# karapostK/hassaku

Measured on AMD Instinct MI355X. Metric: BPR triplets/sec, higher is better.
Workload: dtype f32

## Files before the change

hassaku_amd/csrc/hsk_fwd_part.h:

```cpp
#pragma once
#include "hsk_sampler.h"
#include "hsk_sort.h"
#include "hsk_step_kernels.h"

struct hsk_ride_fwd {
  int n_total;
  hsk_ride_sort Bk;
  hsk_ride_sample S;
  hsk_ride_sort R;
};
struct hsk_ride_item {
  int n_total;
  hsk_ride_sort C;
  hsk_ride_sort H;
};

struct hsk_part_args {
  int n_part;
  int n_items;
  int n_ahead_blocks;
  int ahead_stride;
};
#define HSK_PART_LIST_MAX 256

__device__ __forceinline__ void hsk_ride_fwd_roles(const hsk_ride_fwd& rf, int bid) {
  if (bid < rf.Bk.n_blocks) {
    __shared__ int bucket_lds[5 * HSK_PIPE_MAX_IPB + 2];
    hsk_sort_bucket_body(rf.Bk.perm1, rf.Bk.n_entries, rf.Bk.n_items, rf.Bk.plan, rf.Bk.bstart, rf.Bk.perm, rf.Bk.offsets,
                         nullptr, nullptr, bid, bucket_lds);
    return;
  }
  bid -= rf.Bk.n_blocks;
  if (bid < rf.S.n_blocks) {
    hsk_ride_sample_body(rf.S, bid);
    return;
  }
  bid -= rf.S.n_blocks;
  if (bid < rf.R.n_blocks) hsk_sort_rowscan_body(rf.R.hist, rf.R.plan, rf.R.btot, bid);
}

template <int V, int NCH, bool FULL, int R, int LOSS, bool GEN>
__global__ __launch_bounds__(256) void k_fwd_part(const float* __restrict__ Uw, const float* __restrict__ Iw,
                                                  const float* __restrict__ Ib, const int* __restrict__ u32,
                                                  const int* __restrict__ it32, int B, int K , int D, float inv_norm,
                                                  float* __restrict__ g_s, float* __restrict__ dUp,
                                                  double* __restrict__ loss_p, hsk_lazy_user_args lz, hsk_part_args pa,
                                                  hsk_ahead_args aa, hsk_ride_fwd rf) {
  static_assert(LOSS == HSK_LOSS_BPR || LOSS == HSK_LOSS_BCE, "the sampled softmax needs all negatives in one wave");
  int bid = (int)blockIdx.x;
  if (bid < rf.n_total) {
    hsk_ride_fwd_roles(rf, bid);
    return;
  }
  bid -= rf.n_total;
  if (pa.ahead_stride > 0) {
    const int o = bid >> 3, r = bid & 7, n_ao = pa.n_ahead_blocks >> 3;
    const int period = pa.ahead_stride + 1, full = n_ao * period;
    if (o < full) {
      const int k = o / period, j = o - k * period;
      if (j == pa.ahead_stride) {
        hsk_user_ahead_body<V, NCH, FULL, GEN>(aa, k * 8 + r);
        return;
      }
      bid = (k * pa.ahead_stride + j) * 8 + r;
    } else {
      bid = (n_ao * pa.ahead_stride + (o - full)) * 8 + r;
    }
  } else {
    if (bid < pa.n_ahead_blocks) {
      hsk_user_ahead_body<V, NCH, FULL, GEN>(aa, bid);
      return;
    }
    bid -= pa.n_ahead_blocks;
  }
  const int lane = hsk_lane();
  const int wave = hsk_uniform_i(threadIdx.x >> 6);
  const int P = pa.n_part, M = 8 / P;
  const int xcd = bid & 7, q = xcd / M, sx = xcd - q * M, t = bid >> 3;
  const int b = (t * M + sx) * 4 + wave;
  if (b >= B) return;

  using Row = hsk_row<V, NCH>;
  const int* __restrict__ irow = it32 + (long long)b * K;
  const int u_v = u32[b];
  const int i0_v = irow[0];
  int idv[HSK_PART_LIST_MAX / 64];
#pragma unroll
  for (int r = 0; r < HSK_PART_LIST_MAX / 64; ++r) {
    const int c = P + r * 64 + lane;
    idv[r] = (c < K) ? irow[c] : -1;
  }
  const int u = hsk_uniform_i(u_v);
  const int i0 = hsk_uniform_i(i0_v);
  Row ur, r0, acc;
  hsk_row_load<V, NCH, FULL>(ur, Uw + (long long)u * D, lane, D);
  hsk_row_load<V, NCH, FULL>(r0, Iw + (long long)i0 * D, lane, D);
  int done_v = 0, own_v = 0;
  if (lz.mU) {
    done_v = lz.last_step[u];
    own_v = lz.owner[u];
  }
  const float bias0 = Ib ? Ib[i0] : 0.f;
  __shared__ int lst_id[4][HSK_PART_LIST_MAX], lst_col[4][HSK_PART_LIST_MAX];
  const int lo = (int)(((long long)q * pa.n_items + P - 1) / P), hi = (int)(((long long)(q + 1) * pa.n_items + P - 1) / P);
  int n_mine = 0;
#pragma unroll
  for (int r = 0; r < HSK_PART_LIST_MAX / 64; ++r) {
    const bool mine = idv[r] >= lo && idv[r] < hi;
    const unsigned long long m = __ballot(mine);
    if (mine) {
      const int pos = n_mine + __popcll(m & ((1ull << lane) - 1ull));
      lst_id[wave][pos] = idv[r];
      lst_col[wave][pos] = P + r * 64 + lane;
    }
    n_mine += __popcll(m);
  }
  __builtin_amdgcn_wave_barrier();

  int kc = 0;
  int nr = min(64, n_mine);
  int myidx = (lane < nr) ? lst_id[wave][lane] : i0;
  int mycol = (lane < nr) ? lst_col[wave][lane] : 0;
  Row bufA[R], bufB[R];
  auto prefetch = [&](Row(&buf)[R], int j) {
#pragma unroll
    for (int r = 0; r < R; ++r)
      if (j + r < nr)
        hsk_row_load<V, NCH, FULL>(buf[r], Iw + (long long)hsk_readlane_i(myidx, j + r) * D, lane, D);
  };
  prefetch(bufA, 0);
  float mybias = Ib ? Ib[myidx] : 0.f;

  if (lz.mU)
    hsk_user_row_current<V, NCH, FULL>(ur, u, b, B, D, lane, lz, q == 0, hsk_uniform_i(done_v), hsk_uniform_i(own_v));
  else if (lz.ucur && q == 0)
    hsk_row_store<V, NCH, FULL>(ur, lz.ucur + (long long)b * D, lane, D);
  hsk_row_zero(acc);
  const float s0 = hsk_wave_sum(hsk_row_dot_partial(ur, r0)) + bias0;

  float gsum = 0.f;
  double lsum = 0.0;
  while (true) {
    float gv = 0.f, xv = 0.f;
    auto process = [&](Row(&buf)[R], int j) {
      hsk_weigh_rows<LOSS>(ur, buf, j, nr, lane, mybias, s0, inv_norm, acc, gsum, gv, xv);
    };
    for (int j = 0; j < nr; j += 2 * R) {
      prefetch(bufB, j + R);
      process(bufA, j);
      prefetch(bufA, j + 2 * R);
      process(bufB, j + R);
    }
    if (lane < nr) {
      g_s[(long long)b * K + mycol] = gv;
      lsum += (double)hsk_softplus(LOSS == HSK_LOSS_BPR ? -xv : xv);
    }
    kc += 64;
    if (kc >= n_mine) break;
    nr = min(64, n_mine - kc);
    myidx = (lane < nr) ? lst_id[wave][kc + lane] : i0;
    mycol = (lane < nr) ? lst_col[wave][kc + lane] : 0;
    prefetch(bufA, 0);
    mybias = Ib ? Ib[myidx] : 0.f;
  }
  float gp;
  if (LOSS == HSK_LOSS_BPR) {
    gp = gsum;
  } else {
    gp = (q == 0) ? inv_norm / (1.f + expf(s0)) : 0.f;
    if (q == 0 && lane == 0) lsum += (double)hsk_softplus(-s0);
  }
  hsk_row_axpy(acc, -gp, r0);
  hsk_row_store<V, NCH, FULL>(acc, dUp + ((long long)b * P + q) * D, lane, D);
  const double l = hsk_wave_sum_f64(lsum);
  if (lane == 0) {
    g_s[(long long)b * K + q] = -gp;
    loss_p[(long long)q * B + b] = l;
  }
}
```

hassaku_amd/csrc/hsk_item_sliced.h:

```cpp
#pragma once
#include "hsk_rows.h"
#include "hsk_step_kernels.h"
#include "hsk_fwd_part.h"

#ifndef HSK_ITEM_MLP
#define HSK_ITEM_MLP 4
#endif
#ifndef HSK_ITEM_NT
#define HSK_ITEM_NT 0
#endif
template <int VS>
__device__ __forceinline__ hsk_vec<VS> hsk_ldg_stream(const float* p) {
#if HSK_ITEM_NT
  hsk_vec<VS> r;
#pragma unroll
  for (int i = 0; i < VS; ++i) r.v[i] = __builtin_nontemporal_load(p + i);
  return r;
#else
  return hsk_ldg<VS>(p);
#endif
}
template <int VS>
__device__ __forceinline__ void hsk_stg_stream(float* p, const hsk_vec<VS>& x) {
#if HSK_ITEM_NT
#pragma unroll
  for (int i = 0; i < VS; ++i) __builtin_nontemporal_store(x.v[i], p + i);
#else
  hsk_stg<VS>(p, x);
#endif
}

#ifdef HSK_DEBUG_XCC
__device__ unsigned hsk_dbg_xcc[64];
#endif
struct hsk_item_args {
  const float* Uw;
  float* Iw; float* Ib; float* mI; float* vI; float* mIb; float* vIb;
  const int* u32;
  const float* g_s; const int* perm; const int* offsets;
  int n_items, K, D, n_slices_pad, items_per_wave;
  hsk_adamw_consts c;
  float* gI_out; float* gIb_out;
  const int* touched; const int* n_touched; int* last_step_i; int step;
  const int* pend;
  const hsk_step_desc* desc; int rel;
  const float2* ctab; int ctab_len;
  int n_part;
};

template <bool PART>
__device__ __forceinline__ float hsk_entry_weight(const hsk_item_args& a, int e, int bpos) {
  float g = a.g_s[e];
  if (PART && e == bpos * a.K)
    for (int q = 1; q < a.n_part; ++q) g += a.g_s[e + q];
  return g;
}

template <bool APPLY, int VS, bool GEN, bool LAZY, bool PART = false>
__device__ __forceinline__ void hsk_item_sliced_body(const hsk_item_args& a, int bid) {
  const float* __restrict__ Uw = a.Uw;
  float* __restrict__ Iw = a.Iw;
  float* __restrict__ Ib = a.Ib;
  float* __restrict__ mI = a.mI;
  float* __restrict__ vI = a.vI;
  float* __restrict__ mIb = a.mIb;
  float* __restrict__ vIb = a.vIb;
  const int* __restrict__ u32 = a.u32;
  const float* __restrict__ g_s = a.g_s;
  const int* __restrict__ perm = a.perm;
  const int* __restrict__ offsets = a.offsets;
  const int n_items = a.n_items, K = a.K, D = a.D, n_slices_pad = a.n_slices_pad, items_per_wave = a.items_per_wave;
  hsk_adamw_consts c = a.c;
  int step = a.step;
  hsk_resolve_step(a.desc, a.rel, a.ctab, a.ctab_len, step, c);
  float* __restrict__ gI_out = a.gI_out;
  float* __restrict__ gIb_out = a.gIb_out;
  const int* __restrict__ touched = a.touched;
  const int* __restrict__ n_touched = a.n_touched;
  int* __restrict__ last_step_i = a.last_step_i;
  const int lane = hsk_lane();
  const int wave = hsk_uniform_i(threadIdx.x >> 6);
  int slice, group;
  if (n_slices_pad < 8) {
    const int xcd = bid & 7, r = bid >> 3;
    slice = xcd % n_slices_pad;
    group = r * (8 / n_slices_pad) + xcd / n_slices_pad;
  } else {
    slice = bid % n_slices_pad;
    group = bid / n_slices_pad;
  }
  constexpr int SW = 64 * VS;
  const int d = slice * SW + lane * VS;
  const bool live = d < D;
  if (slice * SW >= D) return;
  const int first = (group * 4 + wave) * items_per_wave;
  const int n_list = LAZY ? hsk_uniform_i(*n_touched) : n_items;
  for (int t = 0; t < items_per_wave; ++t) {
    const int idx = first + t;
    if (idx >= n_list) return;
    const int i = LAZY ? hsk_uniform_i(touched[idx]) : idx;
    const int beg = hsk_uniform_i(offsets[i]);
    const int end = hsk_uniform_i(offsets[i + 1]);
    hsk_vec<VS> p = hsk_zero<VS>(), m = hsk_zero<VS>(), v = hsk_zero<VS>();
    if (APPLY && live) {
      p = hsk_ldg_stream<VS>(Iw + (long long)i * D + d);
      m = hsk_ldg_stream<VS>(mI + (long long)i * D + d);
      v = hsk_ldg_stream<VS>(vI + (long long)i * D + d);
    }
    hsk_vec<VS> acc = hsk_zero<VS>();
    float gb_lane = 0.f;
    for (int c0 = beg; c0 < end; c0 += 64) {
      const int nr = min(64, end - c0);
      int myu = 0;
      float myg = 0.f;
      if (lane < nr) {
        const int e = perm[c0 + lane];
        const int bpos = e / K;
        myg = PART ? hsk_entry_weight<true>(a, e, bpos) : g_s[e];
        myu = u32 ? u32[bpos] : bpos;
      }
      gb_lane += myg;
      for (int j = 0; j < nr; j += HSK_ITEM_MLP) {
        hsk_vec<VS> val[HSK_ITEM_MLP];
#pragma unroll
        for (int r = 0; r < HSK_ITEM_MLP; ++r)
          val[r] = (j + r < nr && live) ? hsk_ldg<VS>(Uw + (long long)hsk_readlane_i(myu, min(j + r, 63)) * D + d)
                                        : hsk_zero<VS>();
#pragma unroll
        for (int r = 0; r < HSK_ITEM_MLP; ++r)
          if (j + r < nr) {
            const float g = hsk_readlane_f(myg, j + r);
#pragma unroll
            for (int q = 0; q < VS; ++q) acc.v[q] = fmaf(g, val[r].v[q], acc.v[q]);
          }
      }
    }
    if (APPLY) {
      const int behind = (LAZY && !GEN && a.pend) ? (step - 1) - hsk_uniform_i(a.pend[idx]) : 0;
      for (int r = 0; r < behind; ++r) {
#pragma unroll
        for (int q = 0; q < VS; ++q) {
          m.v[q] = fmaf(c.w1, -m.v[q], m.v[q]);
          v.v[q] = v.v[q] * c.beta2;
        }
      }
      if (live) {
#pragma unroll
        for (int q = 0; q < VS; ++q) hsk_adamw_update<GEN>(p.v[q], m.v[q], v.v[q], acc.v[q], c);
        hsk_stg_stream<VS>(Iw + (long long)i * D + d, p);
        hsk_stg_stream<VS>(mI + (long long)i * D + d, m);
        hsk_stg_stream<VS>(vI + (long long)i * D + d, v);
      }
      if (slice == 0 && Ib) {
        const float gbias = hsk_wave_sum(gb_lane);
        if (lane == 0) {
          float pb = Ib[i], mb = mIb[i], vb = vIb[i];
          for (int r = 0; r < behind; ++r) {
            mb = fmaf(c.w1, -mb, mb);
            vb = vb * c.beta2;
          }
          hsk_adamw_update<GEN>(pb, mb, vb, gbias, c);
          Ib[i] = pb;
          mIb[i] = mb;
          vIb[i] = vb;
        }
      }
      if (LAZY && slice == 0 && lane == 0) last_step_i[i] = step;
    } else {
      if (live) hsk_stg<VS>(gI_out + (long long)i * D + d, acc);
      if (slice == 0 && gIb_out) {
        const float gbias = hsk_wave_sum(gb_lane);
        if (lane == 0) gIb_out[i] = gbias;
      }
    }
  }
}

template <int V, int NCH, bool FULL, bool GEN, bool LAZY>
__device__ __forceinline__ void hsk_item_row_body(const hsk_item_args& a, int bid) {
  const int lane = hsk_lane();
  const int idx = bid * 4 + hsk_uniform_i(threadIdx.x >> 6);
  const int n_list = LAZY ? hsk_uniform_i(*a.n_touched) : a.n_items;
  if (idx >= n_list) return;
  hsk_adamw_consts c = a.c;
  int step = a.step;
  hsk_resolve_step(a.desc, a.rel, a.ctab, a.ctab_len, step, c);
  const int i = LAZY ? hsk_uniform_i(a.touched[idx]) : idx;
  const int D = a.D, K = a.K;
  using Row = hsk_row<V, NCH>;
  const int beg = hsk_uniform_i(a.offsets[i]);
  const int end = hsk_uniform_i(a.offsets[i + 1]);
  float* prow = a.Iw + (long long)i * D;
  float* mrow = a.mI + (long long)i * D;
  float* vrow = a.vI + (long long)i * D;
  Row p, m, v, acc;
  hsk_row_load<V, NCH, FULL>(p, prow, lane, D);
  hsk_row_load<V, NCH, FULL>(m, mrow, lane, D);
  hsk_row_load<V, NCH, FULL>(v, vrow, lane, D);
  float pb = 0.f, mb = 0.f, vb = 0.f;
  if (a.Ib && lane == 0) {
    pb = a.Ib[i];
    mb = a.mIb[i];
    vb = a.vIb[i];
  }
  hsk_row_zero(acc);
  float gb_lane = 0.f;
  for (int c0 = beg; c0 < end; c0 += 64) {
    const int nr = min(64, end - c0);
    int myu = 0;
    float myg = 0.f;
    if (lane < nr) {
      const int e = a.perm[c0 + lane];
      myg = a.g_s[e];
      myu = a.u32 ? a.u32[e / K] : e / K;
    }
    gb_lane += myg;
    for (int j = 0; j < nr; j += 4) {
      Row buf[4];
#pragma unroll
      for (int r = 0; r < 4; ++r)
        if (j + r < nr) hsk_row_load<V, NCH, FULL>(buf[r], a.Uw + (long long)hsk_readlane_i(myu, min(j + r, 63)) * D, lane, D);
#pragma unroll
      for (int r = 0; r < 4; ++r)
        if (j + r < nr) hsk_row_axpy(acc, hsk_readlane_f(myg, j + r), buf[r]);
    }
  }
  const int behind = (LAZY && !GEN && a.pend) ? (step - 1) - hsk_uniform_i(a.pend[idx]) : 0;
  for (int r = 0; r < behind; ++r) {
#pragma unroll
    for (int cc = 0; cc < NCH; ++cc)
#pragma unroll
      for (int q = 0; q < V; ++q) {
        m.c[cc].v[q] = fmaf(c.w1, -m.c[cc].v[q], m.c[cc].v[q]);
        v.c[cc].v[q] = v.c[cc].v[q] * c.beta2;
      }
    mb = fmaf(c.w1, -mb, mb);
    vb = vb * c.beta2;
  }
#pragma unroll
  for (int cc = 0; cc < NCH; ++cc)
#pragma unroll
    for (int q = 0; q < V; ++q) hsk_adamw_update<GEN>(p.c[cc].v[q], m.c[cc].v[q], v.c[cc].v[q], acc.c[cc].v[q], c);
  hsk_row_store<V, NCH, FULL>(p, prow, lane, D);
  hsk_row_store<V, NCH, FULL>(m, mrow, lane, D);
  hsk_row_store<V, NCH, FULL>(v, vrow, lane, D);
  if (a.Ib) {
    const float gbias = hsk_wave_sum(gb_lane);
    if (lane == 0) {
      hsk_adamw_update<GEN>(pb, mb, vb, gbias, c);
      a.Ib[i] = pb;
      a.mIb[i] = mb;
      a.vIb[i] = vb;
    }
  }
  if (LAZY && lane == 0) a.last_step_i[i] = step;
}

template <bool APPLY, int VS, bool GEN, bool LAZY = false, bool PART = false>
__global__ __launch_bounds__(256) void k_item_update_sliced(hsk_item_args a, const int* __restrict__ g_ovf = nullptr,
                                                            const int* __restrict__ g_poison = nullptr) {
  if (APPLY && hsk_guard_skip(g_ovf, g_poison)) return;
  hsk_item_sliced_body<APPLY, VS, GEN, LAZY, PART>(a, (int)blockIdx.x);
}

template <int V, int NCH, bool FULL, bool GEN, bool LAZY>
__global__ __launch_bounds__(256) void k_item_update_rows(hsk_item_args a, const int* __restrict__ g_ovf = nullptr,
                                                          const int* __restrict__ g_poison = nullptr) {
  if (hsk_guard_skip(g_ovf, g_poison)) return;
  hsk_item_row_body<V, NCH, FULL, GEN, LAZY>(a, (int)blockIdx.x);
}

template <int V, int NCH, bool FULL, int VS, bool GEN, bool LAZYI, bool PART = false>
__global__ __launch_bounds__(256) __attribute__((amdgpu_waves_per_eu(8, 8)))
void k_item_user(hsk_item_args ia, hsk_user_lazy_args ua, int n_user_blocks, int dense_users, hsk_ahead_args aa,
                 int n_ahead_blocks, hsk_ride_item ri = hsk_ride_item{}) {
  int bid = (int)blockIdx.x;
  if (PART) {
    if (bid < ri.n_total) {
      __shared__ int ride_lds[HSK_SORT_SCATTER_LDS];
      if (bid < ri.C.n_blocks) {
        hsk_sort_scatter_body(ri.C.it32, ri.C.n_entries, ri.C.plan, ri.C.hist, ri.C.btot, ri.C.perm1, ri.C.bstart, bid, ride_lds);
      } else if (bid - ri.C.n_blocks < ri.H.n_blocks) {
        hsk_sort_hist_body(ri.H.it32, ri.H.n_entries, ri.H.plan, ri.H.hist, bid - ri.C.n_blocks, ride_lds);
      }
      return;
    }
    bid -= ri.n_total;
  }
  if (bid < n_user_blocks) {
    if (dense_users)
      hsk_user_update_dense_body<V, NCH, FULL, GEN, PART>(ua, bid);
    else
      hsk_user_update_lazy_body<V, NCH, FULL, GEN, PART>(ua, bid);
    return;
  }
  if (LAZYI && bid < n_user_blocks + n_ahead_blocks) {
    hsk_user_ahead_body<V, NCH, FULL, GEN>(aa, bid - n_user_blocks);
    return;
  }
#ifdef HSK_DEBUG_XCC
  if (threadIdx.x == 0) {
    unsigned xcc;
    asm volatile("s_getreg_b32 %0, hwreg(HW_REG_XCC_ID)" : "=s"(xcc));
    atomicAdd(&hsk_dbg_xcc[((bid - n_user_blocks) & 7) * 8 + (xcc & 7)], 1u);
  }
#endif
  hsk_item_sliced_body<true, VS, GEN, LAZYI, PART>(ia, bid - n_user_blocks - (LAZYI ? n_ahead_blocks : 0));
}

template <int V, int NCH, bool FULL, bool GEN, bool LAZYI>
__global__ __launch_bounds__(256) void k_item_user_small(hsk_item_args ia, hsk_user_lazy_args ua, int n_user_blocks,
                                                         int dense_users, hsk_ahead_args aa, int n_ahead_oct,
                                                         int stride) {
  const int bid = (int)blockIdx.x;
  if (bid < n_user_blocks) {
    if (dense_users)
      hsk_user_update_dense_body<V, NCH, FULL, GEN>(ua, bid);
    else
      hsk_user_update_lazy_body<V, NCH, FULL, GEN>(ua, bid);
    return;
  }
  const int q = (bid - n_user_blocks) >> 3, r = bid & 7;
  int item_oct = q;
  if (n_ahead_oct > 0) {
    const int period = stride + 1, full = n_ahead_oct * period;
    if (q < full) {
      const int k = q / period, j = q - k * period;
      if (j == stride) {
        hsk_user_ahead_body<V, NCH, FULL, GEN>(aa, k * 8 + r);
        return;
      }
      item_oct = k * stride + j;
    } else {
      item_oct = n_ahead_oct * stride + (q - full);
    }
  }
  hsk_item_row_body<V, NCH, FULL, GEN, LAZYI>(ia, item_oct * 8 + r);
}
```

hassaku_amd/csrc/hsk_rows.h:

```cpp
#pragma once
#include "hsk_common.h"
#include <type_traits>

#define HSK_OWNER_NONE 0x7fffffff

struct hsk_step_desc {
  long long start0;
  const int64_t* order;
  int step0;
  int pad;
};

template <typename F>
static int hsk_dispatch_dim(int64_t D, F&& f) {
  int V = (D % 4 == 0) ? 4 : (D % 2 == 0) ? 2 : 1;
  int64_t chunks = hsk_ceil_div(D, (int64_t)64 * V);
  int nch = chunks <= 1 ? 1 : chunks <= 2 ? 2 : chunks <= 4 ? 4 : chunks <= 8 ? 8 : 0;
  if (nch == 0) {
    hsk_set_error("embedding_dim %lld not supported (max %d for this alignment)", (long long)D, 64 * V * 8);
    return HSK_ERR_UNSUPPORTED;
  }
  bool full = (D == (int64_t)64 * V * nch);
#define HSK_CASE(v, n)                                                                          \
  if (V == v && nch == n) {                                                                     \
    if (v == 4 && full)                                                                         \
      return f(std::integral_constant<int, v>{}, std::integral_constant<int, n>{}, std::true_type{}); \
    return f(std::integral_constant<int, v>{}, std::integral_constant<int, n>{}, std::false_type{});  \
  }
  HSK_CASE(4, 1) HSK_CASE(4, 2) HSK_CASE(4, 4) HSK_CASE(4, 8)
  HSK_CASE(2, 1) HSK_CASE(2, 2) HSK_CASE(2, 4) HSK_CASE(2, 8)
  HSK_CASE(1, 1) HSK_CASE(1, 2) HSK_CASE(1, 4) HSK_CASE(1, 8)
#undef HSK_CASE
  hsk_set_error("internal: no kernel for dim %lld", (long long)D);
  return HSK_ERR_UNSUPPORTED;
}

template <int V, int NCH>
struct hsk_row {
  hsk_vec<V> c[NCH];
};

template <int V, int NCH, bool FULL>
__device__ __forceinline__ void hsk_row_load(hsk_row<V, NCH>& r, const float* __restrict__ base, int lane, int D) {
#pragma unroll
  for (int c = 0; c < NCH; ++c) {
    const int off = (c * 64 + lane) * V;
    if (FULL || off < D)
      r.c[c] = hsk_ldg<V>(base + off);
    else
      r.c[c] = hsk_zero<V>();
  }
}

template <int V, int NCH, bool FULL>
__device__ __forceinline__ void hsk_row_store(const hsk_row<V, NCH>& r, float* __restrict__ base, int lane, int D) {
#pragma unroll
  for (int c = 0; c < NCH; ++c) {
    const int off = (c * 64 + lane) * V;
    if (FULL || off < D) hsk_stg<V>(base + off, r.c[c]);
  }
}

template <int V, int NCH>
__device__ __forceinline__ void hsk_row_zero(hsk_row<V, NCH>& r) {
#pragma unroll
  for (int c = 0; c < NCH; ++c) r.c[c] = hsk_zero<V>();
}

template <int V, int NCH>
__device__ __forceinline__ float hsk_row_dot_partial(const hsk_row<V, NCH>& a, const hsk_row<V, NCH>& b) {
  float s = 0.f;
#pragma unroll
  for (int c = 0; c < NCH; ++c)
#pragma unroll
    for (int i = 0; i < V; ++i) s = fmaf(a.c[c].v[i], b.c[c].v[i], s);
  return s;
}

template <int V, int NCH>
__device__ __forceinline__ void hsk_row_axpy(hsk_row<V, NCH>& acc, float a, const hsk_row<V, NCH>& x) {
#pragma unroll
  for (int c = 0; c < NCH; ++c)
#pragma unroll
    for (int i = 0; i < V; ++i) acc.c[c].v[i] = fmaf(a, x.c[c].v[i], acc.c[c].v[i]);
}

template <int V, int NCH>
__device__ __forceinline__ void hsk_row_add(hsk_row<V, NCH>& acc, const hsk_row<V, NCH>& x) {
#pragma unroll
  for (int c = 0; c < NCH; ++c)
#pragma unroll
    for (int i = 0; i < V; ++i) acc.c[c].v[i] += x.c[c].v[i];
}

__device__ __forceinline__ float hsk_softplus(float z) {
  return fmaxf(z, 0.f) + log1pf(expf(-fabsf(z)));
}

template <int LOSS, int V, int NCH, int R>
__device__ __forceinline__ void hsk_weigh_rows(const hsk_row<V, NCH>& ur, const hsk_row<V, NCH> (&buf)[R], int j, int nr,
                                               int lane, float mybias, float s0, float inv_norm, hsk_row<V, NCH>& acc,
                                               float& gsum, float& gv, float& xv) {
  static_assert(LOSS == HSK_LOSS_BPR || LOSS == HSK_LOSS_BCE, "the sampled softmax keeps a running max: row by row");
  if (j >= nr) return;
  float sv = 0.f;
#pragma unroll
  for (int r = 0; r < R; ++r)
    if (j + r < nr) sv = hsk_writelane_f(hsk_wave_sum(hsk_row_dot_partial(ur, buf[r])), j + r, sv);
  const float s = sv + mybias;
  float x, g;
  if (LOSS == HSK_LOSS_BPR) {
    x = s0 - s;
    g = inv_norm / (1.f + expf(x));
  } else {
    x = s;
    g = inv_norm / (1.f + expf(-s));
  }
  const bool mine = lane >= j && lane < min(j + R, nr);
  gv = mine ? g : gv;
  xv = mine ? x : xv;
#pragma unroll
  for (int r = 0; r < R; ++r) {
    if (j + r < nr) {
      const float gr = hsk_readlane_f(g, j + r);
      if (LOSS == HSK_LOSS_BPR) gsum += gr;
      hsk_row_axpy(acc, gr, buf[r]);
    }
  }
}

__device__ __forceinline__ int hsk_clamp_index(long long idx, long long n, int32_t* status) {
  if (idx < 0 || idx >= n) {
    if (status) atomicOr(status, HSK_STATUS_BAD_INDEX);
    return 0;
  }
  return (int)idx;
}
```

Before: 2.462 billion.

## Specialize full-slice item gathers and unguard forward prefetch loop with occupancy hints

The forward partial kernel gets a waves-per-EU attribute chosen from the row register footprint. Its double-buffered negative loop now does unconditional, clamped gathers in the steady state, with a guarded tail that handles the remaining rows, and uses empty asm pins to hold registers in place. The sliced item update gains a WHOLE specialization for dimensions divisible by the slice width. That path drops bounds checks, batch-gathers user rows, and defers the param/moment loads until the first gather. The aim is fewer per-row branches, more memory-level parallelism and better occupancy, at the risk of register spills or extra code size from the added template variants.

After: 2.455 billion. About the same (-0.3%).

```diff
diff --git a/hassaku_amd/csrc/hsk_fwd_part.h b/hassaku_amd/csrc/hsk_fwd_part.h
--- a/hassaku_amd/csrc/hsk_fwd_part.h
+++ b/hassaku_amd/csrc/hsk_fwd_part.h
@@ -40,7 +40,9 @@
 }
 
 template <int V, int NCH, bool FULL, int R, int LOSS, bool GEN>
-__global__ __launch_bounds__(256) void k_fwd_part(const float* __restrict__ Uw, const float* __restrict__ Iw,
+__global__ __launch_bounds__(256)
+__attribute__((amdgpu_waves_per_eu(V * NCH * R <= 12 ? 6 : V * NCH * R <= 24 ? 4 : 1)))
+void k_fwd_part(const float* __restrict__ Uw, const float* __restrict__ Iw,
                                                   const float* __restrict__ Ib, const int* __restrict__ u32,
                                                   const int* __restrict__ it32, int B, int K , int D, float inv_norm,
                                                   float* __restrict__ g_s, float* __restrict__ dUp,
@@ -121,7 +123,7 @@
   int nr = min(64, n_mine);
   int myidx = (lane < nr) ? lst_id[wave][lane] : i0;
   int mycol = (lane < nr) ? lst_col[wave][lane] : 0;
-  Row bufA[R], bufB[R];
+  Row bufA[R];
   auto prefetch = [&](Row(&buf)[R], int j) {
 #pragma unroll
     for (int r = 0; r < R; ++r)
@@ -145,11 +147,24 @@
     auto process = [&](Row(&buf)[R], int j) {
       hsk_weigh_rows<LOSS>(ur, buf, j, nr, lane, mybias, s0, inv_norm, acc, gsum, gv, xv);
     };
-    for (int j = 0; j < nr; j += 2 * R) {
-      prefetch(bufB, j + R);
+    int j = 0;
+    for (; j + 3 * R <= nr; j += 2 * R) {
+      Row bufB[R];
+      hsk_rows_gather<V, NCH, FULL>(bufB, Iw, myidx, j + R, 63, lane, D);
+      hsk_row_pin(ur);
+      hsk_weigh_rows<LOSS>(ur, bufA, j, j + R, lane, mybias, s0, inv_norm, acc, gsum, gv, xv);
+      hsk_row_pin(acc);
+      hsk_rows_gather<V, NCH, FULL>(bufA, Iw, myidx, j + 2 * R, 63, lane, D);
+      hsk_weigh_rows<LOSS>(ur, bufB, j + R, j + 2 * R, lane, mybias, s0, inv_norm, acc, gsum, gv, xv);
+      hsk_row_pin(acc);
+    }
+    if (j < nr) {
+      Row bufC[R];
+      prefetch(bufC, j + R);
       process(bufA, j);
       prefetch(bufA, j + 2 * R);
-      process(bufB, j + R);
+      process(bufC, j + R);
+      process(bufA, j + 2 * R);
     }
     if (lane < nr) {
       g_s[(long long)b * K + mycol] = gv;
diff --git a/hassaku_amd/csrc/hsk_item_sliced.h b/hassaku_amd/csrc/hsk_item_sliced.h
--- a/hassaku_amd/csrc/hsk_item_sliced.h
+++ b/hassaku_amd/csrc/hsk_item_sliced.h
@@ -56,7 +56,7 @@
   return g;
 }
 
-template <bool APPLY, int VS, bool GEN, bool LAZY, bool PART = false>
+template <bool APPLY, int VS, bool GEN, bool LAZY, bool PART = false, bool WHOLE = false>
 __device__ __forceinline__ void hsk_item_sliced_body(const hsk_item_args& a, int bid) {
   const float* __restrict__ Uw = a.Uw;
   float* __restrict__ Iw = a.Iw;
@@ -91,7 +91,7 @@
   }
   constexpr int SW = 64 * VS;
   const int d = slice * SW + lane * VS;
-  const bool live = d < D;
+  const bool live = WHOLE || d < D;
   if (slice * SW >= D) return;
   const int first = (group * 4 + wave) * items_per_wave;
   const int n_list = LAZY ? hsk_uniform_i(*n_touched) : n_items;
@@ -102,11 +102,12 @@
     const int beg = hsk_uniform_i(offsets[i]);
     const int end = hsk_uniform_i(offsets[i + 1]);
     hsk_vec<VS> p = hsk_zero<VS>(), m = hsk_zero<VS>(), v = hsk_zero<VS>();
-    if (APPLY && live) {
+    auto load_pmv = [&]() {
       p = hsk_ldg_stream<VS>(Iw + (long long)i * D + d);
       m = hsk_ldg_stream<VS>(mI + (long long)i * D + d);
       v = hsk_ldg_stream<VS>(vI + (long long)i * D + d);
-    }
+    };
+    if (APPLY && live && (!WHOLE || beg == end)) load_pmv();
     hsk_vec<VS> acc = hsk_zero<VS>();
     float gb_lane = 0.f;
     for (int c0 = beg; c0 < end; c0 += 64) {
@@ -120,6 +121,32 @@
         myu = u32 ? u32[bpos] : bpos;
       }
       gb_lane += myg;
+      if (WHOLE) {
+        asm volatile("" : "+v"(myu), "+v"(myg));
+        if (APPLY && c0 == beg) load_pmv();
+        const float* __restrict__ src = Uw + slice * SW;
+        hsk_row<VS, 1> val[HSK_ITEM_MLP];
+        int j = 0;
+        for (; j + HSK_ITEM_MLP <= nr; j += HSK_ITEM_MLP) {
+          hsk_rows_gather<VS, 1, true>(val, src, myu, j, 63, lane, D);
+#pragma unroll
+          for (int r = 0; r < HSK_ITEM_MLP; ++r) {
+            const float g = hsk_readlane_f(myg, j + r);
+#pragma unroll
+            for (int q = 0; q < VS; ++q) acc.v[q] = fmaf(g, val[r].c[0].v[q], acc.v[q]);
+          }
+        }
+        if (j < nr) {
+          hsk_rows_gather<VS, 1, true>(val, src, myu, j, nr - 1, lane, D);
+#pragma unroll
+          for (int r = 0; r < HSK_ITEM_MLP - 1; ++r) {
+            const bool on = j + r < nr;
+            const float g = hsk_readlane_f(myg, min(j + r, nr - 1));
+#pragma unroll
+            for (int q = 0; q < VS; ++q) acc.v[q] = on ? fmaf(g, val[r].c[0].v[q], acc.v[q]) : acc.v[q];
+          }
+        }
+      } else
       for (int j = 0; j < nr; j += HSK_ITEM_MLP) {
         hsk_vec<VS> val[HSK_ITEM_MLP];
 #pragma unroll
@@ -260,7 +287,10 @@
 __global__ __launch_bounds__(256) void k_item_update_sliced(hsk_item_args a, const int* __restrict__ g_ovf = nullptr,
                                                             const int* __restrict__ g_poison = nullptr) {
   if (APPLY && hsk_guard_skip(g_ovf, g_poison)) return;
-  hsk_item_sliced_body<APPLY, VS, GEN, LAZY, PART>(a, (int)blockIdx.x);
+  if (a.D % (64 * VS) == 0)
+    hsk_item_sliced_body<APPLY, VS, GEN, LAZY, PART, true>(a, (int)blockIdx.x);
+  else
+    hsk_item_sliced_body<APPLY, VS, GEN, LAZY, PART, false>(a, (int)blockIdx.x);
 }
 
 template <int V, int NCH, bool FULL, bool GEN, bool LAZY>
@@ -305,7 +335,11 @@
     atomicAdd(&hsk_dbg_xcc[((bid - n_user_blocks) & 7) * 8 + (xcc & 7)], 1u);
   }
 #endif
-  hsk_item_sliced_body<true, VS, GEN, LAZYI, PART>(ia, bid - n_user_blocks - (LAZYI ? n_ahead_blocks : 0));
+  const int ibid = bid - n_user_blocks - (LAZYI ? n_ahead_blocks : 0);
+  if ((FULL && V == VS) || ia.D % (64 * VS) == 0)
+    hsk_item_sliced_body<true, VS, GEN, LAZYI, PART, true>(ia, ibid);
+  else if (!(FULL && V == VS))
+    hsk_item_sliced_body<true, VS, GEN, LAZYI, PART, false>(ia, ibid);
 }
 
 template <int V, int NCH, bool FULL, bool GEN, bool LAZYI>
diff --git a/hassaku_amd/csrc/hsk_rows.h b/hassaku_amd/csrc/hsk_rows.h
--- a/hassaku_amd/csrc/hsk_rows.h
+++ b/hassaku_amd/csrc/hsk_rows.h
@@ -52,6 +52,14 @@
   }
 }
 
+template <int V, int NCH, bool FULL, int R>
+__device__ __forceinline__ void hsk_rows_gather(hsk_row<V, NCH> (&buf)[R], const float* __restrict__ base, int idxv, int j,
+                                                int last, int lane, int D) {
+#pragma unroll
+  for (int r = 0; r < R; ++r)
+    hsk_row_load<V, NCH, FULL>(buf[r], base + (long long)hsk_readlane_i(idxv, min(j + r, last)) * D, lane, D);
+}
+
 template <int V, int NCH, bool FULL>
 __device__ __forceinline__ void hsk_row_store(const hsk_row<V, NCH>& r, float* __restrict__ base, int lane, int D) {
 #pragma unroll
@@ -65,6 +73,14 @@
 __device__ __forceinline__ void hsk_row_zero(hsk_row<V, NCH>& r) {
 #pragma unroll
   for (int c = 0; c < NCH; ++c) r.c[c] = hsk_zero<V>();
+}
+
+template <int V, int NCH>
+__device__ __forceinline__ void hsk_row_pin(hsk_row<V, NCH>& r) {
+#pragma unroll
+  for (int c = 0; c < NCH; ++c)
+#pragma unroll
+    for (int i = 0; i < V; ++i) asm volatile("" : "+v"(r.c[c].v[i]) : : "memory");
 }
 
 template <int V, int NCH>
```
